# modelscope/FunCodec

Measured on AMD Instinct MI355X. Metric: audio-seconds encoded+decoded per wall-sec, 16k-nq32ds640, higher is better.
Workload: dtype f32; 1 GPU; BASELINE.json configs[1]: encodec 16k-nq32ds640 (57.6M, synthetic seeded checkpoint), run_mod=inference (encode + 32-stage RVQ + decode), 16 x 10 s utterances per GPU in micro-batches of 16, n_q=32; utterances_per_gpu=16, samples_per_utterance=160000, micro_batch=16, global_utterances=16, ranks_seen=1, parallelism=single GPU

## Files before the change

funcodec_amd/csrc/engine.hip:

```cpp
#include <hip/hip_runtime.h>

#include <algorithm>
#include <array>
#include <cmath>
#include <cstdio>
#include <cstring>
#include <map>
#include <memory>
#include <string>
#include <vector>

#include "../../include/funcodec_amd.h"
#include "kernels.h"
#include "rvq_beam_kernels.h"
#include "rvq_rate_kernels.h"
#include "laura_kernels.h"
#include "ragged_kernels.h"
#include "seq_kernels.h"
#include "slots_kernels.h"
#include "stream_kernels.h"

namespace {

thread_local std::string g_err;
// ... 675 lines not shown

void choose_tiling(ConvLayer& L) {
    if (L.M > 64) {
        L.BM = 128; L.BN = 128;
        if (L.small_n && L.M <= 256) { L.BM = 32; L.BN = 128; }
    } else if (L.M > 32) { L.BM = 64; L.BN = 256; }
    else { L.BM = 32; L.BN = 256; }
    {
        auto fits = [&](bool dual) { return fc::conv_slab_fits(L.gk, L.gstride, L.dil, 2, L.BN, L.BM, dual && ceil_div_i(L.M, L.BM) < 3); };
        if (!fits(L.dual) && L.BN == 256) {
            if (L.BM == 32) L.BN = 128;
            else { L.BM = 128; L.BN = 128; }
        }
        if (!fits(L.dual)) {
            if (fits(false)) L.force_plain = true;
            else L.unsupported = true;
        }
    }
    const bool plain = ceil_div_i(L.M, L.BM) >= 3 || L.force_plain;
    const bool dual_eff = L.dual && !plain;
    static const int smalln_lds = fc::ab_knob("FC_SMALLN_LDS", 160);
    const size_t lds_budget = (size_t)((L.small_n && L.M <= 1024) ? smalln_lds : 160 / fc::conv_wgs_per_cu(L.BM)) * 1024;
    int cin_p2 = 2;
    while (cin_p2 < L.cin) cin_p2 *= 2;
    int cc = 2;
    for (;;) {
        const int n = cc * 2;
        if (n > 32 || n > cin_p2 || n * L.gk > 64) break;
        if (!fc::conv_slab_fits(L.gk, L.gstride, L.dil, n, L.BN, L.BM, dual_eff)) break;
        if (fc::conv_lds_bytes_for(L.gk, L.gstride, L.dil, n, L.BM, L.BN, L.cin, plain ? 0 : (L.dual ? 2 : 1), 0) > lds_budget) break;
        cc = n;
    }
    static const int row_env = fc::deploy_switch("FC_ROW", 1);
    L.row = false;
    if (row_env && L.gstride == 1) {
        int best = 0;
        for (int n = 4; n <= 64 && n <= L.cin; n *= 2) {
            if (!fc::conv_row_ok(L.gk, L.gstride, L.dil, n, L.BM, L.BN, L.cin, dual_eff)) continue;
            if (fc::conv_lds_bytes_for(L.gk, L.gstride, L.dil, n, L.BM, L.BN, L.cin, plain ? 0 : (L.dual ? 2 : 1), 1) > lds_budget) continue;
            best = n;
        }
        if (best > cc || (best == cc && !plain)) { L.row = true; cc = best; }
    }
    L.CC = cc;
    L.nchunk = ceil_div_i(L.cin, cc);
    L.Mpad = ceil_div_i(L.M, L.BM) * L.BM;
}

template <typename T>
int upload(fc_engine* e, const std::vector<T>& h, T** out) {
    void* d = nullptr;
    HIP_TRY(hipMalloc(&d, h.size() * sizeof(T) + 16));
    HIP_TRY(hipMemcpy(d, h.data(), h.size() * sizeof(T), hipMemcpyHostToDevice));
    e->dev_allocs.push_back(d);
    *out = (T*)d;
    return 0;
}

int pack_gemm(fc_engine* e, ConvLayer& L, const std::vector<float>& wg , const std::vector<float>& bg) {
    const int mtiles = L.Mpad / L.BM;
    const int wbuf = fc::conv_wbuf_floats(L.gk, L.CC, L.BM);
    std::vector<float> packed((size_t)mtiles * L.nchunk * wbuf, 0.f);
    for (int mt = 0; mt < mtiles; ++mt)
        for (int ch = 0; ch < L.nchunk; ++ch)
            for (int kk = 0; kk < L.gk; ++kk)
                for (int cl = 0; cl < L.CC; ++cl) {
                    const int ci = ch * L.CC + cl;
                    if (ci >= L.cin) continue;
                    float* img = &packed[(size_t)(mt * L.nchunk + ch) * wbuf];
                    for (int mm = 0; mm < L.BM; ++mm) {
                        const int m = mt * L.BM + mm;
                        if (m < L.M) img[fc::conv_pack_index(L.gk, L.CC, L.BM, kk, cl, mm)] = wg[((size_t)m * L.cin + ci) * L.gk + kk];
                    }
                }
    std::vector<float> bpad(L.Mpad, 0.f);
    for (int m = 0; m < L.M; ++m) bpad[m] = bg[m];
    if (upload(e, packed, &L.wt)) return 1;
    if (upload(e, bpad, &L.bias)) return 1;
    if (upload(e, fc::conv_koff_table(L.gk, L.gstride, L.dil, L.CC, L.BN, L.row ? 1 : 0), &L.koff)) return 1;
    return 0;
}

int pack_conv(fc_engine* e, ConvLayer& L) {
    const std::string inner = L.transposed ? ".convtr" : ".conv";
    std::vector<float> folded;
    if (L.wnorm) {
        const auto& V = e->host[L.prefix + inner + ".weight_v"].data;
        const auto& G = e->host[L.prefix + inner + ".weight_g"].data;
        const size_t d0 = L.transposed ? L.cin : L.cout, inner_n = V.size() / d0;
        folded.resize(V.size());
        for (size_t r = 0; r < d0; ++r) {
            double ss = 0.0;
            for (size_t j = 0; j < inner_n; ++j) ss += (double)V[r * inner_n + j] * (double)V[r * inner_n + j];
            const float nrm = (float)sqrt(ss);
            const float sc = G[r] / nrm;
            for (size_t j = 0; j < inner_n; ++j) folded[r * inner_n + j] = V[r * inner_n + j] * sc;
        }
    }
    const auto& W = L.wnorm ? folded : e->host[L.prefix + inner + ".weight"].data;
    const auto& Bv = e->host[L.prefix + inner + ".bias"].data;
    if (!L.transposed) {
        if (pack_gemm(e, L, W, Bv)) return 1;
        if (L.cout == 1 && L.stride == 1) {
            if (upload(e, W, &L.w_plain)) return 1;
            L.bias0 = Bv[0];
        }
    } else {
        const int r = L.stride;
        if (L.k != 2 * r) return fail("ConvTranspose1d with kernel != 2*stride is not supported: " + L.prefix);
        std::vector<float> wg((size_t)L.M * L.cin * 2), bg(L.M);
        for (int co = 0; co < L.cout; ++co)
            for (int p = 0; p < r; ++p) {
                const int m = co * r + p;
                bg[m] = Bv[co];
                for (int ci = 0; ci < L.cin; ++ci) {
                    wg[((size_t)m * L.cin + ci) * 2 + 0] = W[((size_t)ci * L.cout + co) * L.k + p + r];
                    wg[((size_t)m * L.cin + ci) * 2 + 1] = W[((size_t)ci * L.cout + co) * L.k + p];
                }
            }
        if (pack_gemm(e, L, wg, bg)) return 1;
    }
    if (L.has_norm) {
        if (upload(e, e->host[L.prefix + ".norm.weight"].data, &L.gamma)) return 1;
        if (upload(e, e->host[L.prefix + ".norm.bias"].data, &L.beta)) return 1;
    }
    return 0;
}

std::vector<float> folded_conv_weight(fc_engine* e, const ConvLayer& L) {
    const std::string inner = L.transposed ? ".convtr" : ".conv";
    if (!L.wnorm) return e->host[L.prefix + inner + ".weight"].data;
    const auto& V = e->host[L.prefix + inner + ".weight_v"].data;
    const auto& G = e->host[L.prefix + inner + ".weight_g"].data;
    const size_t d0 = L.transposed ? L.cin : L.cout, inner_n = V.size() / d0;
    std::vector<float> folded(V.size());
    for (size_t r = 0; r < d0; ++r) {
        double ss = 0.0;
        for (size_t j = 0; j < inner_n; ++j) ss += (double)V[r * inner_n + j] * (double)V[r * inner_n + j];
        const float sc = G[r] / (float)sqrt(ss);
        for (size_t j = 0; j < inner_n; ++j) folded[r * inner_n + j] = V[r * inner_n + j] * sc;
    }
    return folded;
}

int pack_reshead(fc_engine* e, fc_engine::ResBlock& R) {
    static const int enable = fc::ab_knob("FC_RESHEAD", 1);
    const int C = R.shortcut.cin, hid = R.block1.cout, K = R.block1.k;
    R.fused_head = enable && R.shortcut.cout == C && R.block1.cin == C && fc::reshead_ok(C, hid, R.shortcut.k, K, R.block1.dil, R.block1.stride) &&
                   R.shortcut.has_norm == R.block1.has_norm;
    if (!R.fused_head) return 0;
    const std::vector<float> Wsc = folded_conv_weight(e, R.shortcut), Wb1 = folded_conv_weight(e, R.block1);
    std::vector<float> a((size_t)C * C), b((size_t)K * C * hid);
    for (int m = 0; m < C; ++m)
        for (int c = 0; c < C; ++c) a[(size_t)c * C + m] = Wsc[(size_t)m * C + c];
    for (int h = 0; h < hid; ++h)
        for (int c = 0; c < C; ++c)
            for (int kk = 0; kk < K; ++kk) b[((size_t)kk * C + c) * hid + h] = Wb1[((size_t)h * C + c) * K + kk];
    if (upload(e, a, &R.wsc) || upload(e, b, &R.wb1)) return 1;
    if (upload(e, e->host[R.shortcut.prefix + ".conv.bias"].data, &R.bsc)) return 1;
    if (upload(e, e->host[R.block1.prefix + ".conv.bias"].data, &R.bb1)) return 1;
    return 0;
}


int pack_conv2d(fc_engine* e, ConvLayer& L) {
    const std::vector<float> W = folded_weight_nd(e, L.prefix + ".conv", L.wnorm, (size_t)L.cout);
    const auto& Bv = e->host[L.prefix + ".conv.bias"].data;
    const int C = L.c2d, kf = L.kf, kt = L.k;
    const int cpg = C / L.groups, opg = L.cout / L.groups;
    std::vector<float> wg((size_t)L.cout * kf * C * kt, 0.f);
    for (int m = 0; m < L.cout; ++m)
        for (int cl = 0; cl < cpg; ++cl) {
            const int ci = (m / opg) * cpg + cl;
            for (int a = 0; a < kf; ++a)
                for (int b = 0; b < kt; ++b)
                    wg[((size_t)m * (kf * C) + (size_t)a * C + ci) * kt + b] = W[(((size_t)m * cpg + cl) * kf + a) * kt + b];
        }
    if (pack_gemm(e, L, wg, Bv)) return 1;
    static const int gconv_env = fc::ab_knob("FC_GCONV", 1);
    if (gconv_env && L.groups > 1 && L.dil == 1 && fc::gconv2d_ok(cpg, opg, kf, kt, L.stride) && upload(e, W, &L.w_group)) return 1;
    if (L.cout <= 4 && L.stride == 1 && L.sf == 1 && (L.k == 3 || L.k == 5 || L.k == 7) && upload(e, wg, &L.w_plain)) return 1;
    if (L.has_norm) {
        if (upload(e, e->host[L.prefix + ".norm.weight"].data, &L.gamma)) return 1;
        if (upload(e, e->host[L.prefix + ".norm.bias"].data, &L.beta)) return 1;
    }
    return 0;
}

int pack_convtr2d(fc_engine* e, const ConvLayer& S, std::vector<ConvLayer>& phases) {
    const std::vector<float> W = folded_weight_nd(e, S.prefix + ".convtr", S.wnorm, (size_t)S.c2d);
    const auto& Bv = e->host[S.prefix + ".convtr.bias"].data;
    const int C = S.c2d, cout = S.cout, kf = S.kf, kt = S.k, sf = S.sf, r = S.stride;
    const int cpg = C / S.groups, opg = cout / S.groups;
    for (int p = 0; p < sf; ++p) {
        ConvLayer& L = phases[p];
        std::vector<float> wg((size_t)L.M * L.cin * 2, 0.f), bg(L.M);
        for (int co = 0; co < cout; ++co)
            for (int ph = 0; ph < r; ++ph) {
                const int m = co * r + ph;
                bg[m] = Bv[co];
                for (int rr = 0; rr < 2; ++rr)
                    for (int ci = (co / opg) * cpg; ci < (co / opg + 1) * cpg; ++ci) {
                        const int a = p + (1 - rr) * sf;
                        const float* w = &W[(((size_t)ci * opg + co % opg) * kf + a) * kt];
                        const size_t c1 = (size_t)rr * C + ci;
                        wg[((size_t)m * L.cin + c1) * 2 + 0] = w[ph + r];
                        wg[((size_t)m * L.cin + c1) * 2 + 1] = w[ph];
                    }
            }
        if (pack_gemm(e, L, wg, bg)) return 1;
    }
    ConvLayer& L0 = phases[0];
    static const int gconv_env = fc::ab_knob("FC_GCONV", 1);
    if (gconv_env && S.groups > 1 && fc::gconvtr2d_ok(cpg, opg, r)) {
        if (upload(e, W, &L0.w_group) || upload(e, Bv, &L0.w_plain)) return 1;
    }
    if (S.has_norm) {
        if (upload(e, e->host[S.prefix + ".norm.weight"].data, &L0.gamma)) return 1;
        if (upload(e, e->host[S.prefix + ".norm.bias"].data, &L0.beta)) return 1;
    }
    return 0;
}

int pack_dft(fc_engine* e) {
    const int N = e->arch.n_fft, hop = e->arch.stft_hop, F = N / 2 + 1, taps = ceil_div_i(N, hop);
    std::vector<double> win(N);
    for (int n = 0; n < N; ++n) win[n] = 0.5 - 0.5 * cos(2.0 * M_PI * n / N);
    auto tw_cos = [&](long long k) { k %= N; return (k % (N / 2)) == N / 4 ? 0.0 : cos(2.0 * M_PI * (double)k / N); };
    auto tw_sin = [&](long long k) { k %= N; return (k % (N / 2)) == 0 ? 0.0 : sin(2.0 * M_PI * (double)k / N); };
    {
        ConvLayer& L = e->stft;
        std::vector<float> wg((size_t)2 * F * hop * taps, 0.f), bg(2 * F, 0.f);
        for (int f = 0; f < F; ++f)
            for (int j = 0; j < hop; ++j)
                for (int a = 0; a < taps; ++a) {
                    const int n = a * hop + j;
                    if (n >= N) continue;
                    const long long k = (long long)f * n;
                    wg[((size_t)f * hop + j) * taps + a] = (float)(win[n] * tw_cos(k));
                    wg[((size_t)(F + f) * hop + j) * taps + a] = tw_sin(k) == 0.0 ? 0.f : (float)(-win[n] * tw_sin(k));
                }
        if (pack_gemm(e, L, wg, bg)) return 1;
    }
    {
        ConvLayer& L = e->istft;
        std::vector<float> wg((size_t)hop * 2 * F * taps, 0.f), bg(hop, 0.f);
        for (int j = 0; j < hop; ++j)
            for (int f = 0; f < F; ++f)
                for (int a = 0; a < taps; ++a) {
                    const int n = a * hop + j;
                    if (n >= N) continue;
                    const double cf = (f == 0 || f == N / 2) ? 1.0 : 2.0;
                    const long long k = (long long)f * n;
                    const int ap = taps - 1 - a;
                    wg[((size_t)j * 2 * F + f) * taps + ap] = (float)(win[n] * cf * tw_cos(k) / N);
                    wg[((size_t)j * 2 * F + F + f) * taps + ap] = tw_sin(k) == 0.0 ? 0.f : (float)(-win[n] * cf * tw_sin(k) / N);
                }
        if (pack_gemm(e, L, wg, bg)) return 1;
    }
    std::vector<float> w2(N);
    for (int n = 0; n < N; ++n) w2[n] = (float)((float)win[n] * (float)win[n]);
    if (upload(e, w2, &e->win2)) return 1;
    return 0;
}

int pack_lstm(fc_engine* e, LstmBlock& lb) {
    const int H = lb.H;
    if (H == 0) return 0;
    if (H % 16 != 0) return fail("LSTM width must be a multiple of 16");
    for (int l = 0; l < (int)lb.layers.size(); ++l) {
        const std::string sfx = "_l" + std::to_string(l);
        const auto& Wih = e->host[lb.prefix + ".weight_ih" + sfx].data;
        const auto& Whh = e->host[lb.prefix + ".weight_hh" + sfx].data;
        const auto& bih = e->host[lb.prefix + ".bias_ih" + sfx].data;
        const auto& bhh = e->host[lb.prefix + ".bias_hh" + sfx].data;
        std::vector<float> wih_p((size_t)4 * H * H), whh_p((size_t)4 * H * H), b_p(4 * H);
        for (int mp = 0; mp < 4 * H; ++mp) {
            const int blk = mp / 16, u = (mp % 16) / 4, gate = mp % 4;
            const int orig = gate * H + blk * 4 + u;
            memcpy(&wih_p[(size_t)mp * H], &Wih[(size_t)orig * H], H * sizeof(float));
            memcpy(&whh_p[(size_t)mp * H], &Whh[(size_t)orig * H], H * sizeof(float));
            b_p[mp] = bih[orig] + bhh[orig];
        }
        LstmLayer& L = lb.layers[l];
        if (pack_gemm(e, L.inproj, wih_p, b_p)) return 1;
        if (upload(e, whh_p, &L.whh)) return 1;
        if (l >= 1) {
            std::vector<float> cat((size_t)4 * H * 2 * H);
            for (int mp = 0; mp < 4 * H; ++mp) {
                memcpy(&cat[(size_t)mp * 2 * H], &wih_p[(size_t)mp * H], H * sizeof(float));
                memcpy(&cat[(size_t)mp * 2 * H + H], &whh_p[(size_t)mp * H], H * sizeof(float));
            }
            if (upload(e, cat, &L.wcat)) return 1;
            if (upload(e, b_p, &L.bperm)) return 1;
        }
    }
    return 0;
}

int pack_tf(fc_engine* e, TfBlock& tb) {
    if (tb.C == 0) return 0;
    const int C = tb.C;
    auto H = [&](const std::string& k) -> const std::vector<float>& { return e->host[k].data; };
    for (int l = 0; l < (int)tb.layers.size(); ++l) {
        const std::string p = tb.prefix + ".encoders." + std::to_string(l);
        TfLayer& L = tb.layers[l];
        std::vector<float> W((size_t)3 * C * C), Bv((size_t)3 * C);
        int part = 0;
        for (const char* n : {"linear_q", "linear_k", "linear_v"}) {
            const auto& w = H(p + ".self_attn." + n + ".weight");
// ... 2646 lines not shown
```

funcodec_amd/csrc/kernels.h:

```cpp
#pragma once
#include <hip/hip_runtime.h>
#include <stdint.h>
#include <stdio.h>
#include <stdlib.h>

#include <vector>

namespace fc {

inline int ab_knob(const char* name, int dflt) {
#ifdef FC_AB_KNOBS
    const char* v = getenv(name);
    return v ? atoi(v) : dflt;
#else
    if (getenv(name)) fprintf(stderr, "funcodec_amd: %s is set but ignored by this build (tuning knobs need FC_BUILD_DEFINES=FC_AB_KNOBS)\n", name);
    return dflt;
#endif
}

#ifdef FC_AB_KNOBS
#define FC_ABL(mask_, bits_) ((mask_) & (bits_))
#else
#define FC_ABL(mask_, bits_) (0)
#endif

static inline __host__ __device__ int ceil_div(int a, int b) { return (a + b - 1) / b; }

inline int deploy_switch(const char* name, int dflt) {
    const char* v = getenv(name);
    return v ? atoi(v) : dflt;
}

struct Src {
    const float* ptr = nullptr;
    const float* aff = nullptr;
    const float* div = nullptr;
    int used = 0;
    int ld = 0;
};

struct ConvLaunch {
    Src s0, s1;
    int elu = 0; float alpha = 1.f;
    const float* wt = nullptr;
    const float* bias = nullptr;
    const int* koff = nullptr;
    float* out = nullptr;
    long long out_sB = 0, out_sM = 0, out_sT = 1;
    int B = 0, Cin = 0, Tin = 0;
    int M = 0;
    int Tout = 0;
    int k = 1, stride = 1, padL = 0, padR = 0;
    int dil = 1;
    int pad_zero = 0;
    int up_r = 0, trimL = 0, Tfinal = 0;
    double* partials = nullptr;
    int BM = 128, BN = 128, CC = 2, nchunk = 1;
    int row = 0;
    int xq_Tp = 0;
    int Fo = 1;
    int affC = 0;
    long long in_sB0 = 0, in_sB1 = 0;
    long long out_sF = 0, part_sB0 = 0;
    int store_lo = 0, store_hi = 1 << 30;
    const float* w_plain = nullptr;
    float bias_host0 = 0.f;
};

int conv_nblk(const ConvLaunch& c);
bool conv_cout1_ok(const ConvLaunch& c);
bool conv_fewout_rows(const ConvLaunch& c);
void conv_fewout_name(const ConvLaunch& c, char* buf, size_t n);
size_t conv_lds_bytes(const ConvLaunch& c);
int conv_wbuf_floats(int k, int CC, int BM);
bool conv_quad(int CC);
size_t conv_pack_index(int k, int CC, int BM, int kk, int cl, int mm);
size_t conv_lds_bytes_for(int k, int stride, int dil, int CC, int BM, int BN, int Cin, int ntab, int row, int dma_rounds = -1);
bool conv_row_ok(int k, int stride, int dil, int CC, int BM, int BN, int Cin, bool dual);
bool conv_slab_fits(int k, int stride, int dil, int CC, int BN, int BM, bool dual);
int conv_wgs_per_cu(int BM);
std::vector<int> conv_koff_table(int k, int stride, int dil, int CC, int BN, int row);
hipError_t launch_conv(const ConvLaunch& c, hipStream_t st);
void conv_variant(const ConvLaunch& c, int* mode, int* nu, int* row);

struct ResHeadLaunch {
    Src s0, s1;
    const float *wsc = nullptr, *wb1 = nullptr;
    const float *bsc = nullptr, *bb1 = nullptr;
    float *out_sc = nullptr, *out_b1 = nullptr;
    double *part_sc = nullptr, *part_b1 = nullptr;
    int B = 0, C = 0, T = 0, k = 3, dil = 1, padL = 0, padR = 0;
    float alpha = 1.f;
};
bool reshead_ok(int C, int hid, int k_sc, int k_b1, int dil, int stride);
int reshead_ntiles(int T);
hipError_t launch_reshead(const ResHeadLaunch& c, hipStream_t st);

struct GConvLaunch {
    const float *src0 = nullptr, *aff0 = nullptr, *src1 = nullptr, *aff1 = nullptr;
    const float *w = nullptr, *bias = nullptr;
    float* out = nullptr;
    double* partials = nullptr;
    int B = 0, C = 0, M = 0, G = 1, Tin = 0, Tout = 0, Fo = 0, kf = 1, kt = 1, sf = 1, st = 1, padL = 0, padR = 0, elu = 0;
    float alpha = 1.f;
    long long in_sB = 0, in_sF = 0, out_sB = 0, out_sF = 0;
    const char *guard_lo = nullptr, *guard_hi = nullptr;
    int out_halo = 0;
};
bool gconv2d_ok(int cpg, int opg, int kf, int kt, int st);
bool gconv2d_fuses_halo(int kf, int kt, int st, int Fo, int halo);
int gconv2d_nblk(int Tout, int Fo, int G, int kf);
hipError_t launch_gconv2d(const GConvLaunch& c, hipStream_t st);
bool gconvtr2d_ok(int cpg, int opg, int tr);
int gconvtr2d_nblk(int Tin, int tr, int Fin, int fr);
hipError_t launch_gconvtr2d(const float* z, const float* w, const float* bias, float* out, double* partials, int B, int C, int cout, int Fin,
                            int Tin, int fr, int tr, int f_l, int Fout, int trimL, int Tout, long long out_sB, hipStream_t st,
                            int out_halo = 0 );
hipError_t launch_polyphase_in(const float* wav, const float* div, int B, int T, int hop, int n_fft, int Mp, float* xp, hipStream_t st);
hipError_t launch_stft_feats(const float* spec, int B, int F, int Tp, long long spec_sB, int halo, int C, float* feats, hipStream_t st);
hipError_t launch_feats_relayout(float* eng, float* ref, int B, int C, int F, int Tp, int halo, int to_ref, hipStream_t st);
hipError_t launch_halo_rows(float* buf, int B, int F, int halo, int C, int T, int zero, hipStream_t st);
hipError_t launch_halo_rows_short(float* buf, int B, int F, int halo, int pad, int C, int T, hipStream_t st);
hipError_t launch_combine2d(const float* s0, const float* aff0, int h0, const float* s1, const float* aff1, int h1, int elu, float alpha,
                            int B, int F, int C, int T, float* dst, int hd, hipStream_t st,
                            int halo_mode = 0 );
hipError_t launch_spec_from_dec(const float* dec, const float* aff, int B, int F, int Tp, int halo, int C, float* spec, hipStream_t st);
hipError_t launch_istft_finish(const float* ypoly, const float* win2, int B, int hop, int n_fft, int Mp, int Tp, const float* mul, int out_len,
                               float* wav, hipStream_t st);

hipError_t launch_gn_finalize(const double* partials, int nblk, double count, const float* gamma,
                              const float* beta, int C, float eps, int B, float* aff, hipStream_t st);

bool conv_xq_ok(int Cin, int CC, int k, int stride, int dil, int BM, int BN, int row);
size_t conv_xq_floats(int B, int Cin, int Tp, int BN, int stride, int k, int dil);
hipError_t launch_combine_xq(const Src& s0, const Src& s1, int elu, float alpha, int B, int C, int Tin, int padL, int padR, int pad_zero,
                             float* xq, hipStream_t st);

hipError_t launch_combine(const Src& s0, const Src& s1, int elu, float alpha, const float* mul,
                          int B, int C, int Tsrc, int Tcopy, float* out,
                          long long o_sB, long long o_sC, long long o_sT, hipStream_t st);

hipError_t launch_tanh_range(float* x, size_t n, float range, hipStream_t st);

hipError_t launch_volume(const float* wav , int B, int C, int T, float* scale, hipStream_t st,
                         const int* lens = nullptr);

hipError_t launch_transpose_btd(const float* in, int B, int T, int D, float* out, hipStream_t st);

hipError_t launch_rvq_encode(const float* x, int N, int D, int K, int nq, const float* cb, const float* cb_frag ,
                             const float* enorm,
                             int64_t* codes , float* quant ,
                             float* quant_bdt , float* subq ,
                             int Tf, hipStream_t st, const int* src0  = nullptr,
                             const int* nq_rows = nullptr);

__host__ __device__ inline int q0_source_frame(int t, int Tf) {
    const int half = Tf / 2;
    int j;
    if (Tf == 2 * half) j = t >> 1;
    else {
        const float up = (float)half / (float)Tf;
        j = (int)floorf((float)t * up);
        if (j > half - 1) j = half - 1;
    }
    const float down = (float)Tf / (float)half;
    int s = (int)floorf((float)j * down);
    if (s > Tf - 1) s = Tf - 1;
    return s;
}
hipError_t launch_q0_map(int* map , int B, int Tf, hipStream_t st);
hipError_t launch_rvq_decode(const int64_t* codes, int B, int Tf, int nq, int D, int K, const float* cb,
                             float* emb, float* emb_bdt, unsigned* status, hipStream_t st, const int* nq_rows = nullptr);
hipError_t launch_rvq_codes_sum(const int64_t* codes, int N, int D, int K, int nq, const float* cb, float* quant, float* quant_bdt, float* subq,
                                int Tf, hipStream_t st, const int* nq_rows = nullptr);

#define FC_STATUS_LSTM_TIMEOUT 0
#define FC_STATUS_BAD_CODE 1
#define FC_STATUS_BAD_LENGTH 2
#define FC_STATUS_WORDS 16

#define FC_LSTM_MAX_LAYERS 4
hipError_t launch_lstm_wave(const float* const* w, const float* const* bias, const float* xproj, float* h, float* c,
                            float* y, int B, int H, int T, int L, int s, hipStream_t st, const int* steps = nullptr, int sdiv = 1, int smul = 1);

hipError_t launch_lstm_persist(const float* w0, const float* w1, const float* bias1, const float* xproj, float* state, float* y,
                               int B, int H, int T, unsigned* status, hipStream_t st);
hipError_t launch_overlap_add(const float* const* frames, const int* lens, int n_frames, int B, int L0, int stride, int out_len,
                              float* out, hipStream_t st);
hipError_t debug_timeline(unsigned long long* dst);
hipError_t launch_zero_fill(float* p, size_t n, hipStream_t st);
size_t lstm_persist_state_floats(int B, int H, int T);
size_t lstm_persist_clear_floats(int B, int H);
bool lstm_persist_supported(int B, int H, int L, int device);

}
```

funcodec_amd/csrc/kernels.hip:

```cpp
#include "conv_kernel.h"

namespace fc {

#define FC_CONV_TILE(BM, BN, WM, WN) \
    extern template hipError_t launch_conv_tile<BM, BN, WM, WN>(const ConvLaunch&, const ConvArgs&, dim3, size_t, hipStream_t);
FC_CONV_TILE(128, 128, 2, 2)
FC_CONV_TILE(64, 256, 1, 4)
FC_CONV_TILE(32, 256, 1, 4)
FC_CONV_TILE(32, 128, 1, 4)
#undef FC_CONV_TILE
#define FC_CONV_TILE_Q(BM, BN, WM, WN) \
    extern template hipError_t launch_conv_tile_q<BM, BN, WM, WN>(const ConvLaunch&, const ConvArgs&, dim3, size_t, hipStream_t);
FC_CONV_TILE_Q(128, 128, 2, 2)
FC_CONV_TILE_Q(64, 256, 1, 4)
FC_CONV_TILE_Q(32, 256, 1, 4)
FC_CONV_TILE_Q(32, 128, 1, 4)
#undef FC_CONV_TILE_Q

bool conv_quad(int CC) {
    static const int quad_env = ab_knob("FC_QUAD", 1);
    return quad_env != 0 && CC >= 4 && CC % 4 == 0;
}
static int conv_nquads(int k, int CC) { return (((k * (CC / 4) + 1) / 2) + 1) & ~1; }
static int conv_koff_len(int k, int CC) { return conv_quad(CC) ? ((2 * conv_nquads(k, CC) + 3) & ~3) + 8 : (((k * CC / 2) + 3) & ~3) + 8; }
// ... 783 lines not shown
            float e = elu_f(v, p.alpha);
            if (!FAST) e = ((vm >> 16) & 1u) ? e : 0.f;
            if (has_h) Xe[h_row * RH_XS + OFF + p.padL + h_col] = e;
        }
    };

    f32x16 asc[MT];
    f32x16 ab32;
    f32x4 ab16[2];
    auto init_acc = [&]() __attribute__((always_inline)) {
#pragma unroll
        for (int mt = 0; mt < MT; ++mt)
#pragma unroll
            for (int r = 0; r < 16; ++r) asc[mt][r] = bias_s[mt * 32 + (r & 3) + 8 * (r >> 2) + 4 * hi];
        if (B16) {
#pragma unroll
            for (int j = 0; j < 2; ++j)
#pragma unroll
                for (int r = 0; r < 4; ++r) ab16[j][r] = bias_s[C + 4 * g4 + r];
        } else {
#pragma unroll
            for (int r = 0; r < 16; ++r) ab32[r] = bias_s[C + (r & 3) + 8 * (r >> 2) + 4 * hi];
        }
    };
    const int nl0 = wid * 32;
    using Set0 = std::integral_constant<int, 0>;
    using Set1 = std::integral_constant<int, 1>;
    __syncthreads();
    init_acc();

    auto item = [&](int f, int nitems, int& tile, int& chunk, auto set_tag, auto fast_tag) __attribute__((always_inline)) {
        constexpr bool FAST = decltype(fast_tag)::value;
        stage_item(set_tag, fast_tag);
        if (f + 2 < nitems) load_item(set_tag, fast_tag);
        __syncthreads();
        const int c0 = chunk * RH_CH;
        {
            const float* xb = Xa + hi * RH_XS + OFF + p.padL + nl0 + l31;
            const float* wa = Wsc + (c0 + hi) * C + l31;
#pragma unroll 2
            for (int ks = 0; ks < 16; ++ks) {
                const float bv = xb[2 * ks * RH_XS];
#pragma unroll
                for (int mt = 0; mt < MT; ++mt)
                    asc[mt] = __builtin_amdgcn_mfma_f32_32x32x2f32(wa[2 * ks * C + mt * 32], bv, asc[mt], 0, 0, 0);
            }
        }
        if (B16) {
#pragma unroll 1
            for (int kk = 0; kk < K3; ++kk) {
                const float* xb = Xe + g4 * RH_XS + OFF + nl0 + r16 + kk * p.dil;
                const float* wa = Wb1 + (kk * C + c0 + g4) * HID + r16;
#pragma unroll 4
                for (int q = 0; q < 8; ++q) {
                    const float av = wa[4 * q * HID];
                    ab16[0] = __builtin_amdgcn_mfma_f32_16x16x4f32(av, xb[4 * q * RH_XS], ab16[0], 0, 0, 0);
                    ab16[1] = __builtin_amdgcn_mfma_f32_16x16x4f32(av, xb[4 * q * RH_XS + 16], ab16[1], 0, 0, 0);
                }
            }
        } else {
#pragma unroll 1
            for (int kk = 0; kk < K3; ++kk) {
                const float* xb = Xe + hi * RH_XS + OFF + nl0 + l31 + kk * p.dil;
                const float* wa = Wb1 + (kk * C + c0 + hi) * HID + l31;
#pragma unroll 4
                for (int ks = 0; ks < 16; ++ks)
                    ab32 = __builtin_amdgcn_mfma_f32_32x32x2f32(wa[2 * ks * HID], xb[2 * ks * RH_XS], ab32, 0, 0, 0);
            }
        }
        const bool tile_done = chunk == NCH - 1;
        if (tile_done) {
            const int n0 = tile * RH_BN;
            float s1 = 0.f, s2 = 0.f, u1 = 0.f, u2 = 0.f;
            {
                const int col = n0 + nl0 + l31;
                const bool okc = FAST || col < p.T;
                float* o = p.out_sc + ubase + col + (size_t)(4 * hi) * p.T;
#pragma unroll
                for (int mt = 0; mt < MT; ++mt)
#pragma unroll
                    for (int r = 0; r < 16; ++r) {
                        const size_t mo = (size_t)(mt * 32 + (r & 3) + 8 * (r >> 2)) * p.T;
                        const float v = asc[mt][r];
                        if (FAST) { o[mo] = v; s1 += v; s2 = fmaf(v, v, s2); }
                        else if (okc) { o[mo] = v; s1 += v; s2 = fmaf(v, v, s2); }
                    }
            }
            float* ob = p.out_b1 + (size_t)b * HID * p.T;
            if (B16) {
                const int col = n0 + nl0 + r16;
                float* o = ob + col + (size_t)(4 * g4) * p.T;
#pragma unroll
                for (int j = 0; j < 2; ++j) {
#pragma unroll
                    for (int r = 0; r < 4; ++r) {
                        const float v = ab16[j][r];
                        const size_t mo = (size_t)r * p.T + 16 * j;
                        if (FAST) { o[mo] = v; u1 += v; u2 = fmaf(v, v, u2); }
                        else if (col + 16 * j < p.T) { o[mo] = v; u1 += v; u2 = fmaf(v, v, u2); }
                    }
                }
            } else {
                const int col = n0 + nl0 + l31;
                float* o = ob + col + (size_t)(4 * hi) * p.T;
#pragma unroll
                for (int r = 0; r < 16; ++r) {
                    const float v = ab32[r];
                    const size_t mo = (size_t)((r & 3) + 8 * (r >> 2)) * p.T;
                    if (FAST) { o[mo] = v; u1 += v; u2 = fmaf(v, v, u2); }
                    else if (col < p.T) { o[mo] = v; u1 += v; u2 = fmaf(v, v, u2); }
                }
            }
            if (p.part_sc) {
                const float w0 = wave_sum_f32(s1), w1 = wave_sum_f32(s2), w2 = wave_sum_f32(u1), w3 = wave_sum_f32(u2);
                if (lane == 0) *(f32x4*)(red + 4 * wid) = (f32x4){w0, w1, w2, w3};
            }
            init_acc();
        }
        __syncthreads();
        if (tile_done) {
            if (p.part_sc && tid < 4) {
                const int outp = tid >> 1, comp = tid & 1;
                double* dst = outp ? p.part_b1 : p.part_sc;
                const float* rr = red + outp * 2 + comp;
                dst[((size_t)b * p.ntiles + tile) * 2 + comp] = (((double)rr[0] + (double)rr[4]) + (double)rr[8]) + (double)rr[12];
            }
            ++tile; chunk = 0;
        } else {
            ++chunk;
        }
    };
    auto run = [&](int ta, int tb, auto fast_tag) __attribute__((always_inline)) {
        if (ta >= tb) return;
        const int nitems = (tb - ta) * NCH;
        ld_tile = ta; ld_chunk = 0; st_chunk = 0;
        int tile = ta, chunk = 0;
        load_item(Set0(), fast_tag);
        if (nitems > 1) load_item(Set1(), fast_tag);
        for (int f = 0; f < nitems; f += 2) {
            item(f, nitems, tile, chunk, Set0(), fast_tag);
            if (f + 1 < nitems) item(f + 1, nitems, tile, chunk, Set1(), fast_tag);
        }
    };
    int e0 = (p.padL + RH_BN - 1) / RH_BN;
    int e1 = p.T - p.padR - RH_BN >= 0 ? (p.T - p.padR - RH_BN) / RH_BN + 1 : 0;
    if (e1 < e0) e1 = e0;
    const int f0 = e0 < t_begin ? t_begin : (e0 > t_end ? t_end : e0);
    const int f1 = e1 < f0 ? f0 : (e1 > t_end ? t_end : e1);
    run(t_begin, f0, std::false_type());
    run(f0, f1, std::true_type());
    run(f1, t_end, std::false_type());
}

size_t reshead_lds_bytes(int C, int K3) {
    const int HID = C / 2;
    return (size_t)(C * C + K3 * C * HID + 2 * RH_CH * RH_XS + C + HID + 16) * sizeof(float);
}
int reshead_ntiles(int T) { return ceil_div(T, RH_BN); }
bool reshead_ok(int C, int hid, int k_sc, int k_b1, int dil, int stride) {
    return (C == 32 || C == 64) && hid * 2 == C && k_sc == 1 && stride == 1 && (k_b1 == 3 || k_b1 == 5 || k_b1 == 7) && (k_b1 - 1) * dil <= 8;
}

template <int C, int K3, bool DUAL>
static hipError_t launch_reshead_t(const ResHeadArgs& a, dim3 grid, size_t lds, hipStream_t st) {
    static std::atomic<unsigned long long> attr_done{0ull};
    auto kfn = reshead_kernel<C, K3, DUAL>;
    int dev = 0;
    (void)hipGetDevice(&dev);
    const unsigned long long bit = 1ull << (dev & 63);
    if (!(attr_done.load(std::memory_order_acquire) & bit)) {
        hipError_t ea = hipFuncSetAttribute((const void*)kfn, hipFuncAttributeMaxDynamicSharedMemorySize, 160 * 1024);
        if (ea != hipSuccess) return ea;
        attr_done.fetch_or(bit, std::memory_order_release);
    }
    hipLaunchKernelGGL(kfn, grid, dim3(256), lds, st, a);
    return hipGetLastError();
}

hipError_t launch_reshead(const ResHeadLaunch& c, hipStream_t st) {
    if (!reshead_ok(c.C, c.C / 2, 1, c.k, c.dil, 1)) return hipErrorInvalidValue;
    ResHeadArgs a;
    a.src0 = c.s0.ptr; a.aff0 = c.s0.aff; a.src1 = c.s1.ptr; a.aff1 = c.s1.aff;
    a.wsc = c.wsc; a.wb1 = c.wb1; a.bsc = c.bsc; a.bb1 = c.bb1;
    a.out_sc = c.out_sc; a.out_b1 = c.out_b1; a.part_sc = c.part_sc; a.part_b1 = c.part_b1;
    a.T = c.T; a.padL = c.padL; a.padR = c.padR; a.dil = c.dil;
    const int maxpad = c.padL > c.padR ? c.padL : c.padR;
    a.Leff = c.T > maxpad ? c.T : maxpad + 1;
    a.ntiles = reshead_ntiles(c.T);
    a.alpha = c.alpha;
    const size_t lds = reshead_lds_bytes(c.C, c.k);
    const int per_cu = (int)((160 * 1024) / lds) > 3 ? 3 : (int)((160 * 1024) / lds);
    static const int target_env = ab_knob("FC_RH_WGS", 0);
    const int target = target_env ? target_env : 256 * (per_cu < 1 ? 1 : per_cu);
    int G = target / c.B;
    if (G < 1) G = 1;
    if (G > a.ntiles) G = a.ntiles;
    dim3 grid(G, c.B);
    const bool dual = c.s1.ptr != nullptr;
#define FC_RH(CC, KK)                                                                              \
    if (c.C == CC && c.k == KK)                                                                    \
        return dual ? launch_reshead_t<CC, KK, true>(a, grid, lds, st) : launch_reshead_t<CC, KK, false>(a, grid, lds, st);
    FC_RH(32, 3) FC_RH(64, 3) FC_RH(32, 5) FC_RH(64, 5) FC_RH(32, 7) FC_RH(64, 7)
#undef FC_RH
    return hipErrorInvalidValue;
}

__global__ __launch_bounds__(256) void gn_finalize_kernel(const double* __restrict__ partials, int nblk, double count,
                                                          const float* __restrict__ gamma, const float* __restrict__ beta,
                                                          int C, float eps, float* __restrict__ aff) {
    __shared__ double sh[2][256];
    const int b = blockIdx.x, tid = threadIdx.x;
    double s1 = 0.0, s2 = 0.0;
    for (int i = tid; i < nblk; i += 256) {
        s1 += partials[((size_t)b * nblk + i) * 2];
        s2 += partials[((size_t)b * nblk + i) * 2 + 1];
    }
    sh[0][tid] = s1; sh[1][tid] = s2;
    __syncthreads();
    for (int o = 128; o >= 1; o >>= 1) {
        if (tid < o) { sh[0][tid] += sh[0][tid + o]; sh[1][tid] += sh[1][tid + o]; }
        __syncthreads();
    }
    const double mean = sh[0][0] / count;
    double var = sh[1][0] / count - mean * mean;
    if (var < 0.0) var = 0.0;
    const float rstd = (float)(1.0 / sqrt(var + (double)eps));
    const float meanf = (float)mean;
    for (int c = tid; c < C; c += 256) {
        const float a = rstd * gamma[c];
        const float s = fmaf(-a, meanf, beta[c]);
        ((float2*)aff)[(size_t)b * C + c] = make_float2(a, s);
    }
}

hipError_t launch_gn_finalize(const double* partials, int nblk, double count, const float* gamma, const float* beta,
                              int C, float eps, int B, float* aff, hipStream_t st) {
    hipLaunchKernelGGL(gn_finalize_kernel, dim3(B), dim3(256), 0, st, partials, nblk, count, gamma, beta, C, eps, aff);
    return hipGetLastError();
}

__global__ __launch_bounds__(256) void combine_kernel(Src s0, Src s1, int elu, float alpha, const float* __restrict__ mul,
                                                      int C, int Tsrc, int Tcopy, float* __restrict__ out,
                                                      long long o_sB, long long o_sC, long long o_sT) {
    const int b = blockIdx.z, c = blockIdx.y;
    const size_t row = (size_t)b * C + c;
    float2 a0 = make_float2(1.f, 0.f), a1 = make_float2(1.f, 0.f);
    if (s0.aff) a0 = ((const float2*)s0.aff)[row];
    if (s1.ptr && s1.aff) a1 = ((const float2*)s1.aff)[row];
    const float m = mul ? mul[b] : 1.f;
    if (o_sT == 1 && !s0.div) {
        float* orow = out + (size_t)b * o_sB + (size_t)c * o_sC;
        const float* r0 = s0.ptr + row * Tsrc;
        const float* r1 = s1.ptr ? s1.ptr + row * Tsrc : r0;
        const int T4 = Tcopy >> 2;
        for (int q = blockIdx.x * 256 + threadIdx.x; q < T4; q += gridDim.x * 256) {
            const f32x4 x0 = *(const f32x4u*)(r0 + 4 * q);
            const f32x4 x1 = s1.ptr ? (f32x4)(*(const f32x4u*)(r1 + 4 * q)) : x0;
            f32x4 y;
#pragma unroll
            for (int j = 0; j < 4; ++j) {
                float v = x0[j];
                if (s0.aff) v = fmaf(v, a0.x, a0.y);
                if (s1.ptr) {
                    float w = x1[j];
                    if (s1.aff) w = fmaf(w, a1.x, a1.y);
                    v = v + w;
                }
                if (elu) v = elu_f(v, alpha);
                if (mul) v = v * m;
                y[j] = v;
            }
            *(f32x4u*)(orow + 4 * q) = y;
        }
        for (int t = 4 * T4 + blockIdx.x * 256 + threadIdx.x; t < Tcopy; t += gridDim.x * 256) {
            float v = r0[t];
            if (s0.aff) v = fmaf(v, a0.x, a0.y);
            if (s1.ptr) {
                float w = r1[t];
                if (s1.aff) w = fmaf(w, a1.x, a1.y);
                v = v + w;
            }
            if (elu) v = elu_f(v, alpha);
            if (mul) v = v * m;
            orow[t] = v;
        }
        return;
    }
    for (int t = blockIdx.x * 256 + threadIdx.x; t < Tcopy; t += gridDim.x * 256) {
        float v = s0.ptr[row * Tsrc + t];
        if (s0.div) v = v / s0.div[b];
        if (s0.aff) v = fmaf(v, a0.x, a0.y);
        if (s1.ptr) {
            float w = s1.ptr[row * Tsrc + t];
            if (s1.aff) w = fmaf(w, a1.x, a1.y);
            v = v + w;
        }
        if (elu) v = elu_f(v, alpha);
        if (mul) v = v * m;
        out[(size_t)b * o_sB + (size_t)c * o_sC + (size_t)t * o_sT] = v;
    }
}

hipError_t launch_combine(const Src& s0, const Src& s1, int elu, float alpha, const float* mul, int B, int C, int Tsrc,
                          int Tcopy, float* out, long long o_sB, long long o_sC, long long o_sT, hipStream_t st) {
    if (Tcopy <= 0 || B <= 0) return hipSuccess;
    int gx = ceil_div(Tcopy, 256 * 4);
    if (gx < 1) gx = 1;
    hipLaunchKernelGGL(combine_kernel, dim3(gx, C, B), dim3(256), 0, st, s0, s1, elu, alpha, mul, C, Tsrc, Tcopy, out,
                       o_sB, o_sC, o_sT);
    return hipGetLastError();
}

__global__ __launch_bounds__(256) void combine_xq_kernel(Src s0, Src s1, int elu, float alpha, int C, int Tin, int padL, int padR, int pad_zero,
                                                         int Leff, float* __restrict__ xq) {
    const int b = blockIdx.z, g4 = blockIdx.y, Tp = padL + Tin + padR;
    const size_t row0 = (size_t)b * C + 4 * g4;
    float2 a0[4], a1[4];
#pragma unroll
    for (int s4 = 0; s4 < 4; ++s4) {
        a0[s4] = s0.aff ? ((const float2*)s0.aff)[row0 + s4] : make_float2(1.f, 0.f);
        a1[s4] = (s1.ptr && s1.aff) ? ((const float2*)s1.aff)[row0 + s4] : make_float2(1.f, 0.f);
    }
    const float* r0 = s0.ptr + row0 * Tin;
    const float* r1 = s1.ptr ? s1.ptr + row0 * Tin : r0;
    f32x4* orow = (f32x4*)xq + ((size_t)b * (C >> 2) + g4) * (size_t)Tp;
    const int hi_lim = Tin + padR, refl = 2 * (Leff - 1);
    auto act = [&](float v, float w, int s4) __attribute__((always_inline)) {
        if (s0.aff) v = fmaf(v, a0[s4].x, a0[s4].y);
        if (s1.ptr) v = v + (s1.aff ? fmaf(w, a1[s4].x, a1[s4].y) : w);
        if (elu) v = elu_f(v, alpha);
        return v;
    };
    const int T4 = (Tp + 3) >> 2;
    for (int q = blockIdx.x * 256 + threadIdx.x; q < T4; q += gridDim.x * 256) {
        const int g = 4 * q - padL;
        f32x4 x0[4], x1[4];
        bool ok[4] = {true, true, true, true};
        if (g >= 0 && g + 3 < Tin) {
#pragma unroll
            for (int s4 = 0; s4 < 4; ++s4) {
                x0[s4] = *(const f32x4u*)(r0 + (size_t)s4 * Tin + g);
                x1[s4] = s1.ptr ? (f32x4)(*(const f32x4u*)(r1 + (size_t)s4 * Tin + g)) : x0[s4];
            }
        } else {
#pragma unroll
            for (int j = 0; j < 4; ++j) {
                const int gj = g + j;
                bool o = gj >= -padL && gj < hi_lim;
                int src = gj < 0 ? -gj : gj;
                src = src >= Leff ? refl - src : src;
                if (pad_zero) { src = gj; o = o && gj >= 0; }
// ... 156 lines not shown
```

Measured before the change: 10700 audio-s/s.

## Add MFMA quad-layout reshead kernel for C=64 residual block heads

Adds a specialized residual-head kernel for C=64 that computes the shortcut 1x1 conv and the first block conv with 32x32x2 f32 MFMA instructions. Weights are repacked on the host into a quad-interleaved layout, and activations are staged in LDS in the same layout. For k=3 without a dual input, the shortcut weights are held in registers, which shrinks LDS use. Loads are double-buffered across channel halves. The goal is to cut ALU and LDS cost in the fused shortcut+block1 head, at the price of heavier register pressure (launch_bounds 256,2) and more complex indexing.

```diff
diff --git a/funcodec_amd/csrc/engine.hip b/funcodec_amd/csrc/engine.hip
--- a/funcodec_amd/csrc/engine.hip
+++ b/funcodec_amd/csrc/engine.hip
@@ -851,10 +851,10 @@
     const std::vector<float> Wsc = folded_conv_weight(e, R.shortcut), Wb1 = folded_conv_weight(e, R.block1);
     std::vector<float> a((size_t)C * C), b((size_t)K * C * hid);
     for (int m = 0; m < C; ++m)
-        for (int c = 0; c < C; ++c) a[(size_t)c * C + m] = Wsc[(size_t)m * C + c];
+        for (int c = 0; c < C; ++c) a[fc::reshead_wsc_index(C, c, m)] = Wsc[(size_t)m * C + c];
     for (int h = 0; h < hid; ++h)
         for (int c = 0; c < C; ++c)
-            for (int kk = 0; kk < K; ++kk) b[((size_t)kk * C + c) * hid + h] = Wb1[((size_t)h * C + c) * K + kk];
+            for (int kk = 0; kk < K; ++kk) b[fc::reshead_wb1_index(C, K, kk, c, h)] = Wb1[((size_t)h * C + c) * K + kk];
     if (upload(e, a, &R.wsc) || upload(e, b, &R.wb1)) return 1;
     if (upload(e, e->host[R.shortcut.prefix + ".conv.bias"].data, &R.bsc)) return 1;
     if (upload(e, e->host[R.block1.prefix + ".conv.bias"].data, &R.bb1)) return 1;
diff --git a/funcodec_amd/csrc/kernels.h b/funcodec_amd/csrc/kernels.h
--- a/funcodec_amd/csrc/kernels.h
+++ b/funcodec_amd/csrc/kernels.h
@@ -94,6 +94,8 @@
 };
 bool reshead_ok(int C, int hid, int k_sc, int k_b1, int dil, int stride);
 int reshead_ntiles(int T);
+size_t reshead_wsc_index(int C, int c, int m);
+size_t reshead_wb1_index(int C, int k, int kk, int c, int h);
 hipError_t launch_reshead(const ResHeadLaunch& c, hipStream_t st);
 
 struct GConvLaunch {
diff --git a/funcodec_amd/csrc/kernels.hip b/funcodec_amd/csrc/kernels.hip
--- a/funcodec_amd/csrc/kernels.hip
+++ b/funcodec_amd/csrc/kernels.hip
@@ -959,9 +959,294 @@
     run(f1, t_end, std::false_type());
 }
 
-size_t reshead_lds_bytes(int C, int K3) {
+constexpr int RH_PQ = RH_XS + 1;
+constexpr bool reshead_wreg(int k3, bool dual) { return !dual && k3 == 3; }
+
+template <int K3, bool DUAL>
+__global__ __launch_bounds__(256, 2) void reshead_quad_kernel(const ResHeadArgs p) {
+    constexpr int C = 64, HID = 32, NG = C / 8, MT = 2;
+    constexpr bool WREG = reshead_wreg(K3, DUAL);
+    extern __shared__ __attribute__((aligned(16))) float smem[];
+    float* Wb1 = smem;
+    float* Wsc = Wb1 + K3 * C * HID;
+    float* Xa = Wsc + (WREG ? 0 : C * C);
+    float* Xe = Xa + 8 * RH_PQ * 4;
+    float* bias_s = Xe + 8 * RH_PQ * 4;
+    float* red = bias_s + C + HID;
+    float2* aff_s = (float2*)(red + 16);
+
+    const int tid = threadIdx.x, lane = tid & 63, wid = tid >> 6;
+    const int hi = lane >> 5, l31 = lane & 31;
+    const int b = blockIdx.y;
+    const int t_begin = (int)(((long long)p.ntiles * blockIdx.x) / gridDim.x);
+    const int t_end = (int)(((long long)p.ntiles * (blockIdx.x + 1)) / gridDim.x);
+    if (t_begin >= t_end) return;
+
+    for (int i = tid * 4; i < K3 * C * HID; i += 1024) *(f32x4*)(Wb1 + i) = *(const f32x4*)(p.wb1 + i);
+    if (!WREG)
+        for (int i = tid * 4; i < C * C; i += 1024) *(f32x4*)(Wsc + i) = *(const f32x4*)(p.wsc + i);
+    for (int i = tid; i < C + HID; i += 256) bias_s[i] = i < C ? p.bsc[i] : p.bb1[i - C];
+    f32x4 wr[2][4][WREG ? MT : 1];
+    if (WREG) {
+#pragma unroll
+        for (int g = 0; g < NG; ++g)
+#pragma unroll
+            for (int mt = 0; mt < MT; ++mt) wr[g >> 2][g & 3][WREG ? mt : 0] = ((const f32x4*)p.wsc)[(g * 2 + hi) * C + mt * 32 + l31];
+    }
+
+    const int halo = (K3 - 1) * p.dil;
+    const int OFF = (4 - (p.padL & 3)) & 3;
+    const int P = tid & 7, c4 = tid >> 3;
+    const int row0 = 8 * (P >> 1) + (P & 1);
+    const bool has_h = tid < RH_CH * halo;
+    const int h_row = has_h ? tid / halo : 0, h_j = has_h ? tid - h_row * halo : 0;
+    const int h_col = has_h ? (h_j < p.padL ? h_j - p.padL : RH_BN + (h_j - p.padL)) : 0;
+    const int h_lds = ((2 * (h_row >> 3) + (h_row & 1)) * RH_PQ + OFF + p.padL + h_col) * 4 + ((h_row >> 1) & 3);
+    const size_t ubase = (size_t)b * C * p.T;
+    const float* s0 = p.src0 + ubase;
+    const float* s1 = DUAL ? p.src1 + ubase : s0;
+    for (int i = tid; i < (DUAL ? 2 : 1) * C; i += 256) {
+        const float* t = i < C ? p.aff0 : p.aff1;
+        aff_s[i] = t ? ((const float2*)t)[(size_t)b * C + (i & (C - 1))] : make_float2(1.f, 0.f);
+    }
+    const int refl = 2 * (p.Leff - 1);
+    auto resolve = [&](int g, bool& ok) __attribute__((always_inline)) {
+        ok = g >= -p.padL && g < p.T + p.padR;
+        int src = g < 0 ? -g : g;
+        src = src >= p.Leff ? refl - src : src;
+        ok = ok && src >= 0 && src < p.T;
+        return ok ? src : 0;
+    };
+
+    f32x4 v0[2][4], v1[2][DUAL ? 4 : 1];
+    float hv0[2] = {0.f, 0.f}, hv1[2] = {0.f, 0.f};
+    unsigned vmask[2] = {0u, 0u};
+    int ld_tile = 0;
+    auto load_item = [&](auto set_tag, auto fast_tag) __attribute__((always_inline)) {
+        constexpr int S = decltype(set_tag)::value;
+        constexpr bool FAST = decltype(fast_tag)::value;
+        const int n0 = ld_tile * RH_BN, c0 = S * RH_CH;
+        if (S == 1) ++ld_tile;
+        if (FAST) {
+#pragma unroll
+            for (int r = 0; r < 4; ++r) {
+                const size_t o = (size_t)(c0 + row0 + 2 * r) * p.T + n0 + 4 * c4;
+                v0[S][r] = *(const f32x4u*)(s0 + o);
+                if (DUAL) v1[S][r] = *(const f32x4u*)(s1 + o);
+            }
+            const size_t o = (size_t)(c0 + h_row) * p.T + n0 + h_col;
+            hv0[S] = s0[o];
+            if (DUAL) hv1[S] = s1[o];
+        } else {
+            unsigned vm = 0;
+#pragma unroll
+            for (int r = 0; r < 4; ++r) {
+                const size_t ro = (size_t)(c0 + row0 + 2 * r) * p.T;
+#pragma unroll
+                for (int j = 0; j < 4; ++j) {
+                    bool ok;
+                    const int src = resolve(n0 + 4 * c4 + j, ok);
+                    v0[S][r][j] = s0[ro + src];
+                    if (DUAL) v1[S][r][j] = s1[ro + src];
+                    vm |= (ok ? 1u : 0u) << (4 * r + j);
+                }
+            }
+            bool ok;
+            const int src = resolve(n0 + h_col, ok);
+            const size_t o = (size_t)(c0 + h_row) * p.T + src;
+            hv0[S] = s0[o];
+            if (DUAL) hv1[S] = s1[o];
+            vm |= (ok ? 1u : 0u) << 16;
+            vmask[S] = vm;
+        }
+    };
+    auto stage_item = [&](auto set_tag, auto fast_tag) __attribute__((always_inline)) {
+        constexpr int S = decltype(set_tag)::value;
+        constexpr bool FAST = decltype(fast_tag)::value;
+        const unsigned vm = FAST ? 0x1ffffu : vmask[S];
+        f32x4 xa[4], xe[4];
+#pragma unroll
+        for (int r = 0; r < 4; ++r) {
+            const float2 A = aff_s[S * RH_CH + row0 + 2 * r];
+            const float2 B1 = DUAL ? aff_s[C + S * RH_CH + row0 + 2 * r] : make_float2(1.f, 0.f);
+#pragma unroll
+            for (int j = 0; j < 4; ++j) {
+                float v = fmaf(v0[S][r][j], A.x, A.y);
+                if (DUAL) v = v + fmaf(v1[S][DUAL ? r : 0][j], B1.x, B1.y);
+                float e = elu_f(v, p.alpha);
+                if (!FAST) { const bool ok = (vm >> (4 * r + j)) & 1u; v = ok ? v : 0.f; e = ok ? e : 0.f; }
+                xa[j][r] = v; xe[j][r] = e;
+            }
+        }
+        const int o = (P * RH_PQ + OFF + p.padL + 4 * c4) * 4;
+#pragma unroll
+        for (int j = 0; j < 4; ++j) {
+            *(f32x4*)(Xa + o + 4 * j) = xa[j];
+            *(f32x4*)(Xe + o + 4 * j) = xe[j];
+        }
+        {
+            const float2 A = aff_s[S * RH_CH + h_row];
+            const float2 B1 = DUAL ? aff_s[C + S * RH_CH + h_row] : make_float2(1.f, 0.f);
+            float v = fmaf(hv0[S], A.x, A.y);
+            if (DUAL) v = v + fmaf(hv1[S], B1.x, B1.y);
+            float e = elu_f(v, p.alpha);
+            if (!FAST) e = ((vm >> 16) & 1u) ? e : 0.f;
+            if (has_h) Xe[h_lds] = e;
+        }
+    };
+
+    f32x16 asc[MT];
+    f32x16 ab32;
+    auto init_acc = [&]() __attribute__((always_inline)) {
+#pragma unroll
+        for (int mt = 0; mt < MT; ++mt)
+#pragma unroll
+            for (int r = 0; r < 16; ++r) asc[mt][r] = bias_s[mt * 32 + (r & 3) + 8 * (r >> 2) + 4 * hi];
+#pragma unroll
+        for (int r = 0; r < 16; ++r) ab32[r] = bias_s[C + (r & 3) + 8 * (r >> 2) + 4 * hi];
+    };
+    const int nl0 = wid * 32;
+    using Set0 = std::integral_constant<int, 0>;
+    using Set1 = std::integral_constant<int, 1>;
+    __syncthreads();
+    init_acc();
+
+    auto item = [&](int f, int nitems, int& tile, auto set_tag, auto fast_tag) __attribute__((always_inline)) {
+        constexpr int S = decltype(set_tag)::value;
+        constexpr bool FAST = decltype(fast_tag)::value;
+        stage_item(set_tag, fast_tag);
+        if (f + 2 < nitems) load_item(set_tag, fast_tag);
+        __syncthreads();
+        {
+            const f32x4* xb = (const f32x4*)Xa + hi * RH_PQ + OFF + p.padL + nl0 + l31;
+            const f32x4* wa = (const f32x4*)Wsc + (S * 8 + hi) * C + l31;
+            f32x4 bv[2], av[2][MT];
+            auto feed = [&](auto q_tag, f32x4& bq, f32x4 (&aq)[MT]) __attribute__((always_inline)) {
+                constexpr int q = decltype(q_tag)::value;
+                bq = xb[2 * q * RH_PQ];
+#pragma unroll
+                for (int mt = 0; mt < MT; ++mt) aq[mt] = WREG ? wr[S][q][WREG ? mt : 0] : wa[2 * q * C + mt * 32];
+            };
+            auto mul = [&](const f32x4& bq, const f32x4 (&aq)[MT]) __attribute__((always_inline)) {
+                __builtin_amdgcn_sched_barrier(0);
+#pragma unroll
+                for (int j = 0; j < 4; ++j)
+#pragma unroll
+                    for (int mt = 0; mt < MT; ++mt) asc[mt] = __builtin_amdgcn_mfma_f32_32x32x2f32(aq[mt][j], bq[j], asc[mt], 0, 0, 0);
+                __builtin_amdgcn_sched_barrier(0);
+            };
+            feed(std::integral_constant<int, 0>(), bv[0], av[0]);
+            feed(std::integral_constant<int, 1>(), bv[1], av[1]);
+            mul(bv[0], av[0]);
+            feed(std::integral_constant<int, 2>(), bv[0], av[0]);
+            mul(bv[1], av[1]);
+            feed(std::integral_constant<int, 3>(), bv[1], av[1]);
+            mul(bv[0], av[0]);
+            mul(bv[1], av[1]);
+        }
+        {
+            const f32x4* xb = (const f32x4*)Xe + hi * RH_PQ + OFF + nl0 + l31;
+            const f32x4* wa = (const f32x4*)Wb1 + (S * 8 + hi) * HID + l31;
+            f32x4 bv[2], av[2];
+            auto feed = [&](int i, f32x4& bq, f32x4& aq) __attribute__((always_inline)) {
+                bq = xb[2 * (i & 3) * RH_PQ + (i >> 2) * p.dil];
+                aq = wa[(i >> 2) * (NG * 2 * HID) + 2 * (i & 3) * HID];
+            };
+            auto mul = [&](const f32x4& bq, const f32x4& aq) __attribute__((always_inline)) {
+                __builtin_amdgcn_sched_barrier(0);
+#pragma unroll
+                for (int j = 0; j < 4; ++j) ab32 = __builtin_amdgcn_mfma_f32_32x32x2f32(aq[j], bq[j], ab32, 0, 0, 0);
+                __builtin_amdgcn_sched_barrier(0);
+            };
+            feed(0, bv[0], av[0]);
+#pragma unroll
+            for (int i = 0; i < 4 * K3; i += 2) {
+                feed(i + 1, bv[1], av[1]);
+                mul(bv[0], av[0]);
+                if (i + 2 < 4 * K3) feed(i + 2, bv[0], av[0]);
+                mul(bv[1], av[1]);
+            }
+        }
+        if (S == 1) {
+            const int n0 = tile * RH_BN;
+            float s1 = 0.f, s2 = 0.f, u1 = 0.f, u2 = 0.f;
+            const int col = n0 + nl0 + l31;
+            const bool okc = FAST || col < p.T;
+            {
+                float* o = p.out_sc + ubase + col + (size_t)(4 * hi) * p.T;
+#pragma unroll
+                for (int mt = 0; mt < MT; ++mt)
+#pragma unroll
+                    for (int r = 0; r < 16; ++r) {
+                        const size_t mo = (size_t)(mt * 32 + (r & 3) + 8 * (r >> 2)) * p.T;
+                        const float v = asc[mt][r];
+                        if (FAST) { o[mo] = v; s1 += v; s2 = fmaf(v, v, s2); }
+                        else if (okc) { o[mo] = v; s1 += v; s2 = fmaf(v, v, s2); }
+                    }
+            }
+            {
+                float* o = p.out_b1 + (size_t)b * HID * p.T + col + (size_t)(4 * hi) * p.T;
+#pragma unroll
+                for (int r = 0; r < 16; ++r) {
+                    const float v = ab32[r];
+                    const size_t mo = (size_t)((r & 3) + 8 * (r >> 2)) * p.T;
+                    if (FAST) { o[mo] = v; u1 += v; u2 = fmaf(v, v, u2); }
+                    else if (okc) { o[mo] = v; u1 += v; u2 = fmaf(v, v, u2); }
+                }
+            }
+            if (p.part_sc) {
+                const float w0 = wave_sum_f32(s1), w1 = wave_sum_f32(s2), w2 = wave_sum_f32(u1), w3 = wave_sum_f32(u2);
+                if (lane == 0) *(f32x4*)(red + 4 * wid) = (f32x4){w0, w1, w2, w3};
+            }
+            init_acc();
+        }
+        __syncthreads();
+        if (S == 1) {
+            if (p.part_sc && tid < 4) {
+                const int outp = tid >> 1, comp = tid & 1;
+                double* dst = outp ? p.part_b1 : p.part_sc;
+                const float* rr = red + outp * 2 + comp;
+                dst[((size_t)b * p.ntiles + tile) * 2 + comp] = (((double)rr[0] + (double)rr[4]) + (double)rr[8]) + (double)rr[12];
+            }
+            ++tile;
+        }
+    };
+    auto run = [&](int ta, int tb, auto fast_tag) __attribute__((always_inline)) {
+        if (ta >= tb) return;
+        const int nitems = (tb - ta) * 2;
+        ld_tile = ta;
+        int tile = ta;
+        load_item(Set0(), fast_tag);
+        load_item(Set1(), fast_tag);
+        for (int f = 0; f < nitems; f += 2) {
+            item(f, nitems, tile, Set0(), fast_tag);
+            item(f + 1, nitems, tile, Set1(), fast_tag);
+        }
+    };
+    int e0 = (p.padL + RH_BN - 1) / RH_BN;
+    int e1 = p.T - p.padR - RH_BN >= 0 ? (p.T - p.padR - RH_BN) / RH_BN + 1 : 0;
+    if (e1 < e0) e1 = e0;
+    const int f0 = e0 < t_begin ? t_begin : (e0 > t_end ? t_end : e0);
+    const int f1 = e1 < f0 ? f0 : (e1 > t_end ? t_end : e1);
+    run(t_begin, f0, std::false_type());
+    run(f0, f1, std::true_type());
+    run(f1, t_end, std::false_type());
+}
+
+size_t reshead_lds_bytes(int C, int K3, bool dual) {
     const int HID = C / 2;
+    if (C == 64) return (size_t)(K3 * C * HID + (reshead_wreg(K3, dual) ? 0 : C * C) + 2 * 8 * RH_PQ * 4 + C + HID + 16 + 4 * C) * sizeof(float);
     return (size_t)(C * C + K3 * C * HID + 2 * RH_CH * RH_XS + C + HID + 16) * sizeof(float);
+}
+size_t reshead_wsc_index(int C, int c, int m) {
+    if (C == 64) return ((size_t)((c >> 3) * 2 + (c & 1)) * C + m) * 4 + ((c >> 1) & 3);
+    return (size_t)c * C + m;
+}
+size_t reshead_wb1_index(int C, int k, int kk, int c, int h) {
+    (void)k;
+    const int HID = C / 2;
+    if (C == 64) return ((size_t)((kk * (C / 8) + (c >> 3)) * 2 + (c & 1)) * HID + h) * 4 + ((c >> 1) & 3);
+    return ((size_t)kk * C + c) * HID + h;
 }
 int reshead_ntiles(int T) { return ceil_div(T, RH_BN); }
 bool reshead_ok(int C, int hid, int k_sc, int k_b1, int dil, int stride) {
@@ -971,7 +1256,9 @@
 template <int C, int K3, bool DUAL>
 static hipError_t launch_reshead_t(const ResHeadArgs& a, dim3 grid, size_t lds, hipStream_t st) {
     static std::atomic<unsigned long long> attr_done{0ull};
-    auto kfn = reshead_kernel<C, K3, DUAL>;
+    void (*kfn)(const ResHeadArgs);
+    if constexpr (C == 64) kfn = reshead_quad_kernel<K3, DUAL>;
+    else kfn = reshead_kernel<C, K3, DUAL>;
     int dev = 0;
     (void)hipGetDevice(&dev);
     const unsigned long long bit = 1ull << (dev & 63);
@@ -995,7 +1282,8 @@
     a.Leff = c.T > maxpad ? c.T : maxpad + 1;
     a.ntiles = reshead_ntiles(c.T);
     a.alpha = c.alpha;
-    const size_t lds = reshead_lds_bytes(c.C, c.k);
+    const bool dual = c.s1.ptr != nullptr;
+    const size_t lds = reshead_lds_bytes(c.C, c.k, dual);
     const int per_cu = (int)((160 * 1024) / lds) > 3 ? 3 : (int)((160 * 1024) / lds);
     static const int target_env = ab_knob("FC_RH_WGS", 0);
     const int target = target_env ? target_env : 256 * (per_cu < 1 ? 1 : per_cu);
@@ -1003,7 +1291,6 @@
     if (G < 1) G = 1;
     if (G > a.ntiles) G = a.ntiles;
     dim3 grid(G, c.B);
-    const bool dual = c.s1.ptr != nullptr;
 #define FC_RH(CC, KK)                                                                              \
     if (c.C == CC && c.k == KK)                                                                    \
         return dual ? launch_reshead_t<CC, KK, true>(a, grid, lds, st) : launch_reshead_t<CC, KK, false>(a, grid, lds, st);
```

Result: no change. 10740 audio-s/s, median of 6 (+0.4%).
